# ndas7/Parallel-Systems-MPI-TFIDF

Hardware: AMD Instinct MI355X
Metric: corpus GB/s (TF-IDF hot path: tokenize->TF->DF->tf*idf->ordered output) (higher is better)
Workload: dtype u8/u32 (f64 score)

## Files before the change

parallel-systems-mpi-tfidf_amd/csrc/tokcount_sl.hip:

```cpp
#include "dev_common.h"
#include "dev_vocab.h"
#include "kernels.h"

#if defined(SL_ABL_NOVOCAB) || defined(SL_ABL_NOCOUNT) || defined(SL_ABL_NOROUNDS) || defined(SL_ABL_NOWRITE) || \
    defined(SL_ABL_NOALLOC) || defined(SL_ABL_L2C)
#define SL_ABL 1
#else
#define SL_ABL 0
#endif
#ifdef SL_ABL_NOALLOC
#define SL_ABL_ST 0
#else
#define SL_ABL_ST SL_ABL
#endif

namespace {

#ifndef SL_NT
#define SL_NT 256
#endif
constexpr int NT = SL_NT;
constexpr int NWAVE = NT / 64;
#ifndef SL_WGCU
#define SL_WGCU 4
#endif
constexpr int WG_PER_CU = SL_WGCU;
constexpr int WSTEP = 992;
#ifndef SL_TB
#define SL_TB 3584
#endif
constexpr int TB = SL_TB;
constexpr int EPT = TB / NT;
constexpr uint32_t BW = 8;
constexpr uint32_t NB = TB / BW;
constexpr uint32_t WAVE_CLAIMS = (TB - 2 * NT - 64) / NWAVE;
constexpr int GCAP = 256;
constexpr int TLW = 192;
constexpr uint32_t LEN_LONG = 31u;
constexpr uint32_t SLOT_BITS = 25;
constexpr int PMAX = 16;
#ifdef SL_STAMPS
constexpr int SL_NPH = 12;
#endif

struct SlShared {
    uint32_t TK[TB];
    uint32_t TC[TB];
    int32_t gdoc[GCAP + 1];
    uint32_t dsz[GCAP];
    union {
        struct {
            uint4 stage[NWAVE][64];
            uint32_t tl[NWAVE][TLW];
        } w;
        struct {
            uint32_t dcnt[GCAP];
            uint32_t doff[GCAP];
            uint32_t drun[GCAP];
            uint8_t dstate[GCAP];
        } f;
        struct {
            uint32_t wtot[NWAVE * 4];
            uint4 lrank[NT];
        } q;
    };
    uint4 sel[16];
    uint32_t lbase[8];
    uint32_t fl_nrec, fl_npart;
    uint8_t dpart[GCAP];
    uint8_t dfull[GCAP];
    uint32_t wsum[NWAVE];
    unsigned long long rec_base, part_base;
    unsigned long long next_chunk;
    uint32_t step_next;
};

typedef unsigned int u32x4 __attribute__((ext_vector_type(4)));
typedef unsigned int u32x4u __attribute__((ext_vector_type(4), aligned(1)));

#define RSRC_WORD3 0x00020000

template <int AUX> __device__ __forceinline__ uint4 bload16(__amdgpu_buffer_rsrc_t r, int32_t off) {
    const u32x4 v = __builtin_bit_cast(u32x4, __builtin_amdgcn_raw_buffer_load_b128(r, off, 0, AUX));
    return make_uint4(v.x, v.y, v.z, v.w);
}

__device__ __forceinline__ uint32_t zero_bits(uint32_t x) { return ~(((x & 0x7F7F7F7Fu) + 0x7F7F7F7Fu) | x) & 0x80808080u; }
__device__ __forceinline__ uint32_t compress4(uint32_t m) {
    m >>= 7;
    m |= m >> 7;
    m |= m >> 14;
    return m & 0xFu;
}

__device__ __forceinline__ uint32_t ws_flags4(uint32_t x, uint32_t& lt9) {
    const uint32_t y = x & 0x7F7F7F7Fu;
    const uint32_t a = y + 0x77777777u;
    const uint32_t b = y + 0x72727272u;
    const uint32_t c = (y ^ 0x20202020u) + 0x7F7F7F7Fu;
    lt9 |= ~(a | x) & 0x80808080u;
    return ((a & ~b) | ~c) & ~x & 0x80808080u;
}
__device__ __forceinline__ uint32_t ws_mask16_dot(uint4 v, uint32_t& lt9) {
    const uint32_t f0 = ws_flags4(v.x, lt9), f1 = ws_flags4(v.y, lt9);
    const uint32_t f2 = ws_flags4(v.z, lt9), f3 = ws_flags4(v.w, lt9);
    const uint32_t lo = __builtin_amdgcn_udot4(f0, 0x08040201u, __builtin_amdgcn_udot4(f1, 0x80402010u, 0u, false), false);
    const uint32_t hi = __builtin_amdgcn_udot4(f2, 0x08040201u, __builtin_amdgcn_udot4(f3, 0x80402010u, 0u, false), false);
    return (lo + (hi << 8)) >> 7;
}

__device__ __forceinline__ uint32_t outside16(int32_t pos, int32_t lo, int32_t hi) {
    const int32_t a = lo - pos, b = hi - pos;
    const uint32_t am = a <= 0 ? 0u : (a >= 16 ? 0xFFFFu : ((1u << a) - 1u));
    const uint32_t bm = b <= 0 ? 0u : (b >= 16 ? 0xFFFFu : ((1u << b) - 1u));
    return ~(bm & ~am) & 0xFFFFu;
}

__device__ __forceinline__ uint32_t bkt_hash(uint32_t key) {
    return __umulhi(key * 0x9E3779B1u, NB);
}
struct BktK {
    uint4 a, b;
};
__device__ __forceinline__ uint32_t bkt_slot(uint32_t b, uint32_t j) { return BW * b + j; }
__device__ __forceinline__ BktK bkt_read(const uint32_t* TK, uint32_t b) {
    const uint4* t = reinterpret_cast<const uint4*>(TK) + 2 * b;
    BktK k;
    k.a = t[0];
    k.b = t[1];
    return k;
}
__device__ __forceinline__ uint32_t bkt_match(const BktK& kk, uint32_t key) {
    uint32_t j = kk.a.x == key ? 0u : kk.a.y == key ? 1u : kk.a.z == key ? 2u : kk.a.w == key ? 3u : 8u;
    if (j == 8u) j = kk.b.x == key ? 4u : kk.b.y == key ? 5u : kk.b.z == key ? 6u : kk.b.w == key ? 7u : 8u;
    return j;
}
__device__ __forceinline__ uint32_t bkt_occ(const BktK& kk) {
    const uint32_t ta = __builtin_amdgcn_perm(kk.a.y, kk.a.x, 0x0C0C0703u) | __builtin_amdgcn_perm(kk.a.w, kk.a.z, 0x07030C0Cu);
    const uint32_t tb = __builtin_amdgcn_perm(kk.b.y, kk.b.x, 0x0C0C0703u) | __builtin_amdgcn_perm(kk.b.w, kk.b.z, 0x07030C0Cu);
    return __builtin_amdgcn_udot4(ta & 0x80808080u, 0x08040201u,
                                  __builtin_amdgcn_udot4(tb & 0x80808080u, 0x80402010u, 0u, false), false) >> 7;
}
__device__ __forceinline__ uint32_t bkt_pref(uint32_t key) { return (key * 0x85EBCA77u) >> 29; }
__device__ __forceinline__ uint32_t bkt_pick(uint32_t occ, uint32_t p) {
    const uint32_t e = ~occ & 0xFFu;
    const uint32_t r = ((e | (e << 8)) >> p) & 0xFFu;
    return r ? ((p + (uint32_t)__builtin_ctz(r)) & (BW - 1u)) : BW;
}

__device__ __noinline__ void overflow_record(const K1Out* o, uint32_t doc, uint32_t slot) {
    const uint64_t am = __ballot(1);
    const uint32_t rank = __builtin_amdgcn_mbcnt_hi((uint32_t)(am >> 32), __builtin_amdgcn_mbcnt_lo((uint32_t)am, 0u));
    unsigned long long b = 0;
    if (rank == 0u) b = gatomic_add(o->part_alloc, (unsigned long long)__popcll(am));
    const unsigned long long q = (((unsigned long long)(uint32_t)__builtin_amdgcn_readfirstlane((int)(b >> 32)) << 32) |
                                  (uint32_t)__builtin_amdgcn_readfirstlane((int)(uint32_t)b)) + rank;
    if (SL_ABL) return;
    if (q < o->part_cap) { gmem(o->part_doc)[q] = doc; gmem(o->part_slot)[q] = slot; gmem(o->part_cnt)[q] = 1u; }
    else atomicOr(o->status, ST_PART_FULL);
}

__device__ __noinline__ uint32_t bkt_slow(uint32_t* TK, uint32_t* TC, uint8_t* dpart, const K1Out* o, uint32_t key,
                                          uint32_t b, bool over, uint32_t gd0, uint32_t sb) {
    for (int probe = 0, tries = 0; probe < PMAX && tries < 64; ++tries) {
        const BktK kk = bkt_read(TK, b);
        const uint32_t j = bkt_match(kk, key);
        if (j < BW) { atomicAdd(&TC[bkt_slot(b, j)], 1u); return 0u; }
        const uint32_t e = bkt_pick(bkt_occ(kk), bkt_pref(key));
        if (e < BW) {
            if (over) break;
            const uint32_t old = atomicCAS(&TK[bkt_slot(b, e)], 0u, key);
            if (old == 0u || old == key) {
                atomicAdd(&TC[bkt_slot(b, e)], 1u);
                return old == 0u ? 1u : 0u;
            }
            continue;
        }
        b = b + 1 == NB ? 0u : b + 1;
        ++probe;
    }
    const uint32_t rel = (key & 0x7FFFFFFFu) >> sb;
    dpart[rel] = 1;
    overflow_record(o, gd0 + rel, key & ((1u << sb) - 1u));
    return 0u;
}

__device__ __noinline__ uint32_t resolve_slow(const uint8_t* __restrict__ bytes, uint4* keys, uint64_t* reps,
                                              uint64_t mask, uint32_t* status, uint32_t kind, uint32_t k0,
                                              uint32_t k1, uint32_t k2, uint32_t k3, uint64_t p0, uint64_t dend) {
    if (kind == 1u)
        return vocab_insert_s(keys, reps, mask, ((uint64_t)k1 << 32) | k0, ((uint64_t)k3 << 32) | k2, 0, status);
    uint64_t p = p0;
    while (p < dend && !is_ws(bytes[p])) ++p;
    uint64_t n = 0;
    while (p0 + n < p && bytes[p0 + n] != 0) ++n;
    uint64_t klo, khi;
    if (n < 16) {
        uint64_t lo = 0, hi = 0;
        for (uint32_t k = 0; k < n; ++k) {
            const uint64_t b = bytes[p0 + k];
            if (k < 8) lo |= b << (8 * k); else hi |= b << (8 * (k - 8));
        }
        make_short_key(lo, hi, (uint32_t)n, &klo, &khi);
        return vocab_insert_s(keys, reps, mask, klo, khi, 0, status);
    }
    make_long_key(bytes + p0, n, &klo, &khi);
    if (n > 0xFFFFFFull) atomicOr(status, ST_TERM_LONG);
    const uint64_t rep = ((n < 0xFFFFFFull ? n : 0xFFFFFFull) << 40) | p0;
    return vocab_insert_s(keys, reps, mask, klo, khi, rep, status, bytes);
}

__device__ __forceinline__ void wave_agg_add(uint32_t* ctr, uint32_t idx) {
    const uint32_t i0 = (uint32_t)__builtin_amdgcn_readfirstlane((int)idx);
    const uint64_t am = __ballot(1);
    if (__ballot(idx != i0) == 0ull) {
        if (__builtin_amdgcn_mbcnt_hi((uint32_t)(am >> 32), __builtin_amdgcn_mbcnt_lo((uint32_t)am, 0u)) == 0u)
            atomicAdd(&ctr[i0], (uint32_t)__popcll(am));
    } else {
        atomicAdd(&ctr[idx], 1u);
    }
}
__device__ __forceinline__ uint32_t wave_agg_add_rtn(uint32_t* ctr, uint32_t idx) {
    const uint32_t i0 = (uint32_t)__builtin_amdgcn_readfirstlane((int)idx);
    const uint64_t am = __ballot(1);
    uint32_t k;
    if (__ballot(idx != i0) == 0ull) {
        const uint32_t rank = __builtin_amdgcn_mbcnt_hi((uint32_t)(am >> 32), __builtin_amdgcn_mbcnt_lo((uint32_t)am, 0u));
        uint32_t b = 0;
        if (rank == 0u) b = atomicAdd(&ctr[i0], (uint32_t)__popcll(am));
        k = (uint32_t)__builtin_amdgcn_readfirstlane((int)b) + rank;
    } else {
        k = atomicAdd(&ctr[idx], 1u);
    }
    return k;
}

__device__ __forceinline__ void sl_write_staged(SlShared& S, const K1Out* o, uint32_t gd0, uint32_t sb, uint32_t nrec,
                                                uint32_t npart, unsigned long long rb, unsigned long long pb,
                                                bool rec_ok, bool part_ok) {
    const int tid = threadIdx.x;
    uint32_t* const rec_slot = o->rec_slot;
    uint32_t* const rec_cnt = o->rec_cnt;
    uint32_t* const part_doc = o->part_doc;
    uint32_t* const part_slot = o->part_slot;
    uint32_t* const part_cnt = o->part_cnt;
    const uint32_t smask = (1u << sb) - 1u;
    lds_barrier();
    if (rec_ok && !SL_ABL_ST)
        for (uint32_t i = (uint32_t)tid; i < nrec; i += NT) {
            gmem(rec_slot)[rb + i] = S.TK[i] & smask;
            gmem(rec_cnt)[rb + i] = S.TC[i];
        }
    if (part_ok && !SL_ABL_ST)
        for (uint32_t i = (uint32_t)tid; i < npart; i += NT) {
            const uint32_t k = S.TK[nrec + i];
            gmem(part_doc)[pb + i] = gd0 + ((k & 0x7FFFFFFFu) >> sb);
            gmem(part_slot)[pb + i] = k & smask;
            gmem(part_cnt)[pb + i] = S.TC[nrec + i];
        }
    lds_barrier();
    uint4* t = reinterpret_cast<uint4*>(S.TK);
#pragma unroll
    for (int j = tid; j < 2 * TB / 4; j += NT) t[j] = make_uint4(0, 0, 0, 0);
}

__device__ __forceinline__ void sl_flush(SlShared& S, const K1Out* o, uint32_t gd0, uint32_t ng, uint32_t sb) {
    const int tid = threadIdx.x;
    lds_barrier();
    if (tid < GCAP) { S.f.dcnt[tid] = 0; S.f.drun[tid] = 0; }
    lds_barrier();
    uint32_t ek[EPT], ec[EPT];
#pragma unroll
    for (int j = 0; j < EPT; ++j) {
        ek[j] = S.TK[j * NT + tid];
        ec[j] = S.TC[j * NT + tid];
        if (ek[j]) wave_agg_add(&S.f.dcnt[0], (ek[j] & 0x7FFFFFFFu) >> sb);
    }
    lds_barrier();
    uint32_t packed = 0;
    if ((uint32_t)tid < ng) {
        uint8_t st = 0;
        const uint32_t cnt = S.f.dcnt[tid];
        const bool part = S.dpart[tid] != 0;
        if (cnt) {
            const bool complete = !part && S.dfull[tid] && cnt <= (uint32_t)K5_MAX_PAIRS;
            st = complete ? 2 : 1;
            packed = complete ? cnt : (cnt << 16);
        }
        if ((st == 1 || part) && !SL_ABL) gmem(o->doc_flags)[gd0 + tid] = DF_PARTIAL;
        S.f.dstate[tid] = st;
    }
    uint32_t tot;
    const uint32_t off = block_excl_scan<NT, true>(packed, S.wsum, &tot);
    if ((uint32_t)tid < ng) S.f.doff[tid] = off;
    const uint32_t nrec = tot & 0xFFFFu, npart = tot >> 16;
    if (tid == 0) {
        const unsigned long long rb = (nrec && !SL_ABL) ? gatomic_add(o->rec_alloc, (unsigned long long)nrec) : 0ull;
        if (rb + nrec > o->rec_cap) atomicOr(o->status, ST_REC_FULL);
        S.rec_base = rb;
    } else if (tid == 64) {
        const unsigned long long pb = (npart && !SL_ABL) ? gatomic_add(o->part_alloc, (unsigned long long)npart) : 0ull;
        if (pb + npart > o->part_cap) atomicOr(o->status, ST_PART_FULL);
        S.part_base = pb;
    }
    lds_barrier();
    const unsigned long long rb = S.rec_base, pb = S.part_base;
    const bool rec_ok = rb + nrec <= o->rec_cap, part_ok = pb + npart <= o->part_cap;
    if ((uint32_t)tid < ng && S.f.dstate[tid] == 2) {
        gmem(o->doc_recoff)[gd0 + tid] = rb + (off & 0xFFFFu);
        gmem(o->doc_npairs)[gd0 + tid] = SL_ABL ? 0u : S.f.dcnt[tid];
    }
#pragma unroll
    for (int j = 0; j < EPT; ++j) {
        const uint32_t key = ek[j];
        if (key) {
            const uint32_t rel = (key & 0x7FFFFFFFu) >> sb;
            const uint32_t k = wave_agg_add_rtn(&S.f.drun[0], rel);
            const uint32_t dof = S.f.doff[rel];
            const uint32_t loc = (S.f.dstate[rel] == 2 ? (dof & 0xFFFFu) : nrec + (dof >> 16)) + k;
            S.TK[loc] = key;
            S.TC[loc] = ec[j];
        }
    }
    sl_write_staged(S, o, gd0, sb, nrec, npart, rb, pb, rec_ok, part_ok);
}

constexpr uint32_t FEW = 8;
#ifdef SL_STAMPS
#define SLF_STAMP(k)                                                        \
    do {                                                                    \
        const unsigned long long t_ = __builtin_amdgcn_s_memtime();         \
        st_acc[k] += t_ - st_t;                                             \
        st_t = t_;                                                          \
    } while (0)
#define SLF_ARGS , unsigned long long* st_acc, unsigned long long& st_t
#else
#define SLF_STAMP(k) do {} while (0)
#define SLF_ARGS
#endif
__device__ __forceinline__ void sl_flush_few(SlShared& S, const K1Out* o, uint32_t gd0, uint32_t ng, uint32_t sb SLF_ARGS) {
    const int tid = threadIdx.x;
    const int lane = tid & 63, w = tid >> 6;
    lds_barrier();
    uint32_t ek[EPT], ec[EPT];
    uint32_t c4 = 0;
#pragma unroll
    for (int j = 0; j < EPT; ++j) {
        ek[j] = S.TK[j * NT + tid];
        ec[j] = S.TC[j * NT + tid];
        c4 += (ek[j] >> 31) << (4u * ((ek[j] & 0x7FFFFFFFu) >> sb));
    }
    static_assert(EPT < 16 && FEW == 8, "4-bit per-document entry counts of eight documents");
    uint32_t pk[FEW / 2], inc[FEW / 2];
#pragma unroll
    for (uint32_t q = 0; q < FEW / 2; ++q) {
        pk[q] = ((c4 >> (8u * q)) & 15u) | (((c4 >> (8u * q + 4u)) & 15u) << 16);
        inc[q] = wave_incl_scan(pk[q]);
        if (lane == 63) S.q.wtot[w * (FEW / 2) + q] = inc[q];
    }
    SLF_STAMP(9);
    lds_barrier();
    uint32_t rank[FEW / 2], tot[FEW / 2];
#pragma unroll
    for (uint32_t q = 0; q < FEW / 2; ++q) {
        uint32_t base = 0, t = 0;
#pragma unroll
        for (int k = 0; k < NWAVE; ++k) {
            const uint32_t x = S.q.wtot[k * (FEW / 2) + q];
            base += k < w ? x : 0u;
            t += x;
        }
        rank[q] = base + inc[q] - pk[q];
        tot[q] = t;
    }
    if (w == 0) {
        const uint32_t d = (uint32_t)lane;
        uint32_t cnt = 0, packed = 0;
        uint8_t st = 0;
        if (d < ng) {
#pragma unroll
            for (uint32_t q = 0; q < FEW / 2; ++q)
                if ((d >> 1) == q) cnt = (tot[q] >> (16 * (d & 1u))) & 0xFFFFu;
            const bool part = S.dpart[d] != 0;
            if (cnt) {
                const bool complete = !part && S.dfull[d] && cnt <= (uint32_t)K5_MAX_PAIRS;
                st = complete ? 2 : 1;
                packed = complete ? cnt : (cnt << 16);
            }
            if ((st == 1 || part) && !SL_ABL) gmem(o->doc_flags)[gd0 + d] = DF_PARTIAL;
        }
        const uint32_t incl = wave_incl_scan(packed);
        const uint32_t all = (uint32_t)__builtin_amdgcn_readlane((int)incl, 63);
        const uint32_t off = incl - packed;
        const uint32_t nrec = all & 0xFFFFu, npart = all >> 16;
        unsigned long long a0 = 0, a1 = 0;
        if (lane == 0 && nrec && !SL_ABL) a0 = gatomic_add(o->rec_alloc, (unsigned long long)nrec);
        if (lane == 32 && npart && !SL_ABL) a1 = gatomic_add(o->part_alloc, (unsigned long long)npart);
        const unsigned long long rb = ((unsigned long long)(uint32_t)__builtin_amdgcn_readlane((int)(a0 >> 32), 0) << 32) |
                                      (uint32_t)__builtin_amdgcn_readlane((int)(uint32_t)a0, 0);
        const unsigned long long pb = ((unsigned long long)(uint32_t)__builtin_amdgcn_readlane((int)(a1 >> 32), 32) << 32) |
                                      (uint32_t)__builtin_amdgcn_readlane((int)(uint32_t)a1, 32);
        const bool rec_ok = rb + nrec <= o->rec_cap, part_ok = pb + npart <= o->part_cap;
        if (lane == 0 && !rec_ok) atomicOr(o->status, ST_REC_FULL);
        if (lane == 0 && !part_ok) atomicOr(o->status, ST_PART_FULL);
        if (d < ng && st == 2) {
            gmem(o->doc_recoff)[gd0 + d] = rb + (off & 0xFFFFu);
            gmem(o->doc_npairs)[gd0 + d] = SL_ABL ? 0u : cnt;
        }
        if (d < FEW) S.lbase[d] = d >= ng ? 0u : (st == 2 ? (off & 0xFFFFu) : nrec + (off >> 16));
        if (lane == 0) {
            S.fl_nrec = nrec;
            S.fl_npart = npart;
            S.rec_base = rec_ok ? rb : ~0ull;
            S.part_base = part_ok ? pb : ~0ull;
        }
    }
    lds_barrier();
    SLF_STAMP(10);
    {
        const uint4 lb0 = *reinterpret_cast<const uint4*>(&S.lbase[0]);
        const uint4 lb1 = *reinterpret_cast<const uint4*>(&S.lbase[4]);
        S.q.lrank[tid] = make_uint4(rank[0] + (lb0.x | (lb0.y << 16)), rank[1] + (lb0.z | (lb0.w << 16)),
                                    rank[2] + (lb1.x | (lb1.y << 16)), rank[3] + (lb1.z | (lb1.w << 16)));
    }
    const uint16_t* const lr16 = reinterpret_cast<const uint16_t*>(&S.q.lrank[tid]);
    uint32_t run = 0;
#pragma unroll
    for (int j = 0; j < EPT; ++j) {
        const uint32_t key = ek[j];
        if (key) {
            const uint32_t rel4 = 4u * ((key & 0x7FFFFFFFu) >> sb);
            const uint32_t loc = (uint32_t)lr16[rel4 >> 2] + ((run >> rel4) & 15u);
            run += 1u << rel4;
            S.TK[loc] = key;
            S.TC[loc] = ec[j];
        }
    }
    const unsigned long long rb = S.rec_base, pb = S.part_base;
    sl_write_staged(S, o, gd0, sb, S.fl_nrec, S.fl_npart, rb, pb, rb != ~0ull, pb != ~0ull);
}

#ifdef SL_STAMPS
#define SL_STC , st_cnt
#define SL_STC_ARG , unsigned long long* st_cnt
#else
#define SL_STC
#define SL_STC_ARG
#endif
__device__ __forceinline__ void lds_count(SlShared& S, const K1Out* o, uint32_t key, uint32_t& wclaims, uint32_t gd0,
                                          uint32_t sb SL_STC_ARG) {
    const bool over = wclaims >= WAVE_CLAIMS;
    const uint32_t b = bkt_hash(key);
    const BktK kk = bkt_read(S.TK, b);
    const bool m0 = kk.a.x == key, m1 = kk.a.y == key, m2 = kk.a.z == key, m3 = kk.a.w == key;
    const bool m4 = kk.b.x == key, m5 = kk.b.y == key, m6 = kk.b.z == key, m7 = kk.b.w == key;
    const uint32_t j = ((m1 | m3 | m5 | m7) ? 1u : 0u) | ((m2 | m3 | m6 | m7) ? 2u : 0u) | ((m4 | m5 | m6 | m7) ? 4u : 0u);
    const bool found = m0 | m1 | m2 | m3 | m4 | m5 | m6 | m7;
    const uint32_t pref = bkt_pref(key);
    uint32_t occ = bkt_occ(kk);
    const uint32_t n = bkt_pick(occ, pref);
    const bool hit = key != 0u && found;
    const bool claim = key != 0u && !found && n < BW && !over;
    const uint32_t idx = bkt_slot(b, found ? j : (n & (BW - 1u)));
    const uint32_t old = atomicCAS(&S.TK[idx], hit ? key : (claim ? 0u : 0x7FFFFFFFu), key);
    const bool ok = key != 0u && (old == key || (claim && old == 0u));
    atomicAdd(&S.TC[idx], ok ? 1u : 0u);
    bool claimed = claim && old == 0u;
    bool slow = key != 0u && !ok;
#ifdef SL_STAMPS
    st_cnt[0] += __ballot(slow) != 0ull ? 1u : 0u;
    st_cnt[1] += (uint32_t)__popcll(__ballot(slow));
    st_cnt[2] += (uint32_t)__popcll(__ballot(claim && !ok));
    ++st_cnt[4];
#endif
    uint32_t nn = n;
#pragma unroll
    for (int t = 0; t < 2; ++t) {
        if (claim && slow) {
            occ |= 1u << (nn & (BW - 1u));
            nn = bkt_pick(occ, pref);
        }
        const bool lost = claim && slow && nn < BW;
        if (__ballot(lost) == 0ull) break;
        if (lost) {
            const uint32_t i2 = bkt_slot(b, nn);
            const uint32_t o2 = atomicCAS(&S.TK[i2], 0u, key);
            if (o2 == 0u || o2 == key) {
                atomicAdd(&S.TC[i2], 1u);
                slow = false;
                claimed = o2 == 0u;
            }
        }
    }
    {
        const bool full = slow && !claim && !over && key != 0u;
        if (__ballot(full) != 0ull) {
            if (full) {
                const uint32_t b2 = b + 1u == NB ? 0u : b + 1u;
                const BktK k2 = bkt_read(S.TK, b2);
                const uint32_t j2 = bkt_match(k2, key);
                uint32_t e2 = j2;
                bool ok2 = j2 < BW;
                if (!ok2) {
                    e2 = bkt_pick(bkt_occ(k2), pref);
                    if (e2 < BW) {
                        const uint32_t o2 = atomicCAS(&S.TK[bkt_slot(b2, e2)], 0u, key);
                        ok2 = o2 == 0u || o2 == key;
                        claimed = o2 == 0u;
                    }
                }
                if (ok2) {
                    atomicAdd(&S.TC[bkt_slot(b2, e2)], 1u);
                    slow = false;
                }
            }
        }
    }
#ifdef SL_STAMPS
    st_cnt[3] += __ballot(slow) != 0ull ? 1u : 0u;
    st_cnt[5] += (uint32_t)__popcll(__ballot(slow && claim));
    st_cnt[6] += (uint32_t)__popcll(__ballot(slow && !claim && !over));
    st_cnt[7] += (uint32_t)__popcll(__ballot(slow && over));
#endif
    uint32_t claims = claimed ? 1u : 0u;
    if (__ballot(slow) != 0ull) {
        if (slow) claims = bkt_slow(S.TK, S.TC, S.dpart, o, key, b, over, gd0, sb);
    }
    wclaims += (uint32_t)__popcll(__ballot(claims != 0u));
}

__device__ __forceinline__ uint32_t perm_sel(uint32_t n, uint32_t k) {
    uint32_t s = 0;
    for (uint32_t j = 0; j < 4; ++j) {
        const uint32_t p = 4 * k + j;
        const uint32_t b = p < n ? j : (p == n ? 4u : 12u);
        s |= b << (8 * j);
    }
    return s;
}

struct Round {
    uint32_t k0, k1, k2, k3;
    uint32_t h;
    uint32_t rel, kind;
    int32_t ap;
#ifdef SL_DEBUG
    uint32_t ent;
#endif
    uint4 s0, s1;
};

}

__global__ __launch_bounds__(NT, WG_PER_CU * NT / 256) void k_tokcount_sl(CorpusDev c, const uint64_t* __restrict__ chunk_start,
                                                               const uint32_t* __restrict__ chunk_doc, uint64_t c0,
                                                               uint64_t c1, VocabDev v, const K1Out* __restrict__ o,
                                                               uint32_t sb, uint32_t gcap) {
    __shared__ __attribute__((aligned(16))) SlShared S;
    const int tid = threadIdx.x, lane = tid & 63;
    const int wid = __builtin_amdgcn_readfirstlane(tid >> 6);
    unsigned long long tokens_w = 0;
    bool clean = false;
#ifdef SL_STAMPS
    unsigned long long st_acc[SL_NPH] = {};
    unsigned long long st_t = __builtin_amdgcn_s_memtime(), st_chunks = 0;
    unsigned long long st_cnt[8] = {};
#define SL_STAMP(k)                                                         \
    do {                                                                    \
        const unsigned long long t_ = __builtin_amdgcn_s_memtime();         \
        st_acc[k] += t_ - st_t;                                             \
        st_t = t_;                                                          \
    } while (0)
#else
#define SL_STAMP(k) do {} while (0)
#endif
    if (tid == 0) S.next_chunk = c0 + gatomic_add(o->chunk_ctr, 1ull);
    lds_barrier();
    unsigned long long claim = 0;
    for (uint64_t chunk = (uint64_t)__builtin_amdgcn_readfirstlane((int)(uint32_t)S.next_chunk) |
                          ((uint64_t)__builtin_amdgcn_readfirstlane((int)(uint32_t)(S.next_chunk >> 32)) << 32);
         chunk < c1;) {
    if (tid == 0) claim = c0 + gatomic_add(o->chunk_ctr, 1ull);
    const uint64_t cs = chunk_start[chunk], ce = chunk_start[chunk + 1];
    const uint32_t dfirst = chunk_doc[chunk], dlast = chunk_doc[chunk + 1];
#ifdef SL_STAMPS
    ++st_chunks;
#endif
    if (cs < ce) {

    const uint64_t b0 = cs & ~(uint64_t)15;
    const uint64_t rb = b0 >= 16 ? b0 - 16 : 0;
    const int32_t shift = (int32_t)(b0 - rb);
    const uint64_t avail = c.nbytes > rb ? ((c.nbytes - rb + 15) & ~(uint64_t)15) : 0;
    const __amdgpu_buffer_rsrc_t crs = __builtin_amdgcn_make_buffer_rsrc(
        (void*)(c.bytes + rb), 0, (int)(avail < 0x7FFFFFF0ull ? avail : 0x7FFFFFF0ull), RSRC_WORD3);
    const __amdgpu_buffer_rsrc_t vrs = __builtin_amdgcn_make_buffer_rsrc((void*)v.keys, 0, (int)((v.mask + 1) * 16),
                                                                         RSRC_WORD3);
    const int32_t span = (int32_t)(ce - b0);
    const int32_t cs_rel = (int32_t)(cs - b0);
    const int32_t lo_rel = c.lo > b0 ? (c.lo - b0 > (uint64_t)span ? span : (int32_t)(c.lo - b0)) : -64;
    const int32_t hi_rel = c.hi - b0 > (uint64_t)span + 64 ? span + 64 : (int32_t)(c.hi - b0);

    const uint32_t ng0 = (dlast + 1 - dfirst) < gcap ? (dlast + 1 - dfirst) : gcap;
    const uint64_t dpre = (uint32_t)tid <= ng0 ? c.doc_off[dfirst + tid] : 0ull;
    uint4 pf = bload16<2>(crs, wid * WSTEP + 16 * lane - 16 + shift);
    if (!clean) {
        uint4* t = reinterpret_cast<uint4*>(S.TK);
        for (int j = tid; j < 2 * TB / 4; j += NT) t[j] = make_uint4(0, 0, 0, 0);
        if (tid < 64) {
            const uint32_t n = (uint32_t)tid >> 2, k = (uint32_t)tid & 3u;
            (&S.sel[n].x)[k] = perm_sel(n, k);
        }
        clean = true;
    }
    uint8_t* const stage = reinterpret_cast<uint8_t*>(&S.w.stage[wid][0]);
    uint32_t* const tl = S.w.tl[wid];

    for (uint32_t gd0 = dfirst; gd0 <= dlast; gd0 += gcap) {
        const uint32_t ng = (dlast + 1 - gd0) < gcap ? (dlast + 1 - gd0) : gcap;
        for (uint32_t k = tid; k <= ng; k += NT) {
            const uint64_t d = (gd0 == dfirst && k == (uint32_t)tid) ? dpre : c.doc_off[gd0 + k];
            S.gdoc[k] = d < b0 ? -64 : (d - b0 > (uint64_t)span + 64 ? span + 64 : (int32_t)(d - b0));
        }
        if (tid < GCAP) { S.dsz[tid] = 0; S.dpart[tid] = 0; }
        if (tid == 0) S.step_next = NWAVE;
        lds_barrier();
        if ((uint32_t)tid < ng) S.dfull[tid] = S.gdoc[tid] >= cs_rel && S.gdoc[tid + 1] <= span;
        const int32_t g0 = __builtin_amdgcn_readfirstlane(S.gdoc[0]);
        const int32_t gn = __builtin_amdgcn_readfirstlane(S.gdoc[ng]);
        const int32_t gs = g0 > cs_rel ? g0 : cs_rel;
        const int32_t ge = gn < span ? gn : span;
        SL_STAMP(0);

        Round pend, acc;
        pend.kind = 0;
        pend.k0 = pend.k1 = pend.k2 = pend.k3 = 0;
        pend.h = 0;
        pend.rel = 0;
        pend.ap = 0;
        pend.s0 = pend.s1 = make_uint4(0, 0, 0, 0);
#ifdef SL_DEBUG
        pend.ent = 0;
#endif
        acc = pend;
        uint32_t fill = 0;
        uint32_t wclaims = 0;

        auto promote = [&](Round& p, const Round& a) {
            p.k0 = a.k0; p.k1 = a.k1; p.k2 = a.k2; p.k3 = a.k3;
            p.h = a.h; p.rel = a.rel; p.kind = a.kind; p.ap = a.ap;
#ifdef SL_DEBUG
            p.ent = a.ent;
#endif
#ifdef SL_ABL_NOVOCAB
            p.s0 = make_uint4(p.k0, p.k1, p.k2, p.k3);
            p.s1 = p.s0;
#else
            p.s0 = bload16<0>(vrs, (int32_t)(p.h << 4));
            p.s1 = bload16<0>(vrs, (int32_t)(p.h << 4) + 16);
#endif
        };
        auto finish = [&](const Round& r) {
#ifdef SL_STAMPS
            asm volatile("s_waitcnt vmcnt(0)" ::: "memory");
            SL_STAMP(11);
#endif
            const bool h0 = ((r.s0.x ^ r.k0) | (r.s0.y ^ r.k1) | (r.s0.z ^ r.k2) | (r.s0.w ^ r.k3)) == 0u;
            const bool h1 = ((r.s1.x ^ r.k0) | (r.s1.y ^ r.k1) | (r.s1.z ^ r.k2) | (r.s1.w ^ r.k3)) == 0u;
            uint32_t slot = r.h + (h0 ? 0u : 1u);
#ifdef SL_ABL_NOVOCAB
            const bool need = false;
#else
            const bool need = (r.kind == 2u) | ((r.kind == 1u) & !(h0 | h1));
#endif
            if (__ballot(need) != 0ull) {
                if (need) {
                    const uint64_t p0 = b0 + (uint64_t)(int64_t)r.ap;
                    const uint64_t dend = c.doc_off[gd0 + r.rel + 1];
                    slot = resolve_slow(c.bytes, v.keys, v.rep, v.mask, o->status, r.kind, r.k0, r.k1, r.k2, r.k3, p0,
                                        dend);
                }
            }
            const uint32_t key = (r.kind != 0u && slot != INVALID_SLOT) ? (0x80000000u | (r.rel << sb) | slot) : 0u;
#ifdef SL_DEBUG
            if (o->stamps && r.kind != 0u) {
                const unsigned long long q = atomicAdd(&o->stamps[0], 1ull);
                if (q < (K1_DEBUG_WORDS - 8) / 4) {
                    unsigned long long* d = o->stamps + 8 + 4 * q;
                    d[0] = ((unsigned long long)r.ent << 32) | ((uint32_t)r.ap << 8) | r.kind;
                    d[1] = ((unsigned long long)r.k1 << 32) | r.k0;
                    d[2] = ((unsigned long long)r.k3 << 32) | r.k2;
                    d[3] = ((unsigned long long)key << 32) | slot;
                }
            }
#endif
#ifdef SL_ABL_NOCOUNT
            wclaims += (uint32_t)__popcll(__ballot(key == 0x12345u));
            return;
#endif
            lds_count(S, o, key, wclaims, gd0, sb SL_STC);
        };
        auto build = [&](Round& a, uint32_t e, int32_t sbp) {
            const uint32_t pos = e & 1023u, len = (e >> 10) & 31u;
            a.rel = e >> 16;
            a.ap = sbp - 16 + (int32_t)pos;
            a.kind = len >= 16u ? 2u : 1u;
#ifdef SL_DEBUG
            a.ent = e;
#endif
            const u32x4u raw = *reinterpret_cast<const u32x4u*>(stage + pos);
            const uint4 sl = S.sel[len & 15u];
            a.k0 = __builtin_amdgcn_perm(0x09090909u, raw.x, sl.x);
            a.k1 = __builtin_amdgcn_perm(0x09090909u, raw.y, sl.y);
            a.k2 = __builtin_amdgcn_perm(0x09090909u, raw.z, sl.z);
            a.k3 = __builtin_amdgcn_perm(0x09090909u, raw.w, sl.w);
            a.h = (uint32_t)key_hash(((uint64_t)a.k1 << 32) | a.k0, ((uint64_t)a.k3 << 32) | a.k2) & (uint32_t)v.mask & ~1u;
        };
        auto turn = [&]() {
            finish(pend);
            promote(pend, acc);
            acc.kind = 0u;
            fill = 0u;
        };

        if (gs < ge) {
            const int32_t bs = gs & ~15;
            const int32_t nsteps = (ge - bs + WSTEP - 1) / WSTEP;
            const bool inner_all = bs >= lo_rel + 16 && bs + nsteps * WSTEP + 16 <= hi_rel;
            if (gd0 != dfirst || bs != 0) pf = bload16<2>(crs, bs + wid * WSTEP + 16 * lane - 16 + shift);
            uint32_t wr = 0;
            int32_t wcur = g0, wnext = ng > 1 ? __builtin_amdgcn_readfirstlane(S.gdoc[1]) : gn;
            for (int32_t s = wid, snext = wid; s < nsteps; s = snext) {
                {
                    uint32_t nx = 0;
                    if (lane == 0) nx = atomicAdd(&S.step_next, 1u);
                    snext = __builtin_amdgcn_readfirstlane((int)nx);
                }
                const int32_t sbp = bs + s * WSTEP;
                const int32_t gpos = sbp + 16 * lane - 16;
                const uint4 cur = pf;
#ifdef SL_ABL_L2C
                pf = bload16<2>(crs, bs + (snext & 3) * WSTEP + 16 * lane - 16 + shift);
#else
                pf = bload16<2>(crs, bs + snext * WSTEP + 16 * lane - 16 + shift);
#endif
                reinterpret_cast<uint4*>(stage)[lane] = cur;
                uint32_t lt9 = 0;
                uint32_t ws = ws_mask16_dot(cur, lt9);
                if (!inner_all) ws |= outside16(gpos, lo_rel, hi_rel);
                while (wr + 1 < ng && wnext <= sbp) {
                    ++wr;
                    wcur = wnext;
                    wnext = __builtin_amdgcn_readfirstlane(S.gdoc[wr + 1]);
                }
                uint32_t ds = 0, base = wr;
                const bool multi = wnext < sbp + WSTEP + 16 || wcur + 16 >= sbp;
                if (multi) {
                    for (uint32_t k = wr; k <= ng; ++k) {
                        const int32_t sk = __builtin_amdgcn_readfirstlane(S.gdoc[k]);
                        if (sk >= sbp + WSTEP + 16) break;
                        base += (k > wr && sk < gpos) ? 1u : 0u;
                        if (sk >= gpos && sk < gpos + 16) ds |= 1u << (uint32_t)(sk - gpos);
                    }
                }
                const uint32_t prev = (lane_prev(ws) >> 15) & 1u;
                uint32_t own = (lane >= 1 && lane <= 62) ? 0xFFFFu : 0u;
                if (!(sbp >= gs && sbp + WSTEP <= ge) && own) own &= ~outside16(gpos, gs, ge);
                const uint32_t starts = ~ws & ((ws << 1) | prev | ds) & own & 0xFFFFu;
                uint32_t nul = 0;
                const bool nulany = __ballot(lt9 != 0u) != 0ull;
                if (nulany)
                    nul = compress4(zero_bits(cur.x)) | (compress4(zero_bits(cur.y)) << 4) |
                          (compress4(zero_bits(cur.z)) << 8) | (compress4(zero_bits(cur.w)) << 12);
                const uint32_t stop = ws | ds;
                const uint32_t stop32 = stop | (lane_next(stop) << 16), nul32 = nul | (lane_next(nul) << 16);
                const uint32_t nmine = (uint32_t)__popc(starts);
                const uint32_t incl = wave_incl_scan(nmine);
                const uint32_t ntok = (uint32_t)__builtin_amdgcn_readlane((int)incl, 63);
                SL_STAMP(1);
                if (ntok == 0) continue;
                tokens_w += ntok;
#ifdef SL_ABL_NOROUNDS
                if (!multi && lane == 0) atomicAdd(&S.dsz[wr], ntok);
                continue;
#endif
                if (!multi && lane == 0) atomicAdd(&S.dsz[wr], ntok);
                const bool fast = !multi && !nulany && ntok <= (uint32_t)TLW;
                for (uint32_t tb = 0; tb < ntok; tb += TLW) {
                    if (fast) {
                        const uint32_t eb = ((uint32_t)lane << 4) | (wr << 16), s32 = stop32 | 0x80000000u;
                        uint32_t sm = starts;
                        uint32_t* p = tl + (incl - nmine);
                        while (sm) {
                            const uint32_t i = __builtin_ctz(sm);
                            sm &= sm - 1;
                            *p++ = eb | i | ((uint32_t)__builtin_ctz(s32 >> i) << 10);
                        }
                    } else {
                        uint32_t sm = starts, idx = incl - nmine;
                        while (sm) {
                            const uint32_t i = __builtin_ctz(sm);
                            sm &= sm - 1;
                            if (idx - tb < (uint32_t)TLW) {
                                const uint32_t e = ((stop32 >> i) & ~1u) | (nul32 >> i);
                                const uint32_t len = e ? (uint32_t)__builtin_ctz(e) : LEN_LONG;
                                uint32_t rel = base;
                                if (ds & ((2u << i) - 1u))
                                    while (rel + 1 < ng && S.gdoc[rel + 1] <= gpos + (int32_t)i) ++rel;
                                tl[idx - tb] = ((uint32_t)lane << 4 | i) | ((len < 16u ? len : LEN_LONG) << 10) | (rel << 16);
                                if (multi) atomicAdd(&S.dsz[rel], 1u);
                            }
                            ++idx;
                        }
                    }
                    __builtin_amdgcn_fence(__ATOMIC_RELEASE, "wavefront");
                    __builtin_amdgcn_wave_barrier();
                    __builtin_amdgcn_fence(__ATOMIC_ACQUIRE, "wavefront");
                    const uint32_t cnt = (ntok - tb) < (uint32_t)TLW ? (ntok - tb) : (uint32_t)TLW;
                    SL_STAMP(2);
                    for (uint32_t t = 0; t < cnt;) {
                        const uint32_t m = (64u - fill) < (cnt - t) ? (64u - fill) : (cnt - t);
                        if ((uint32_t)lane >= fill && (uint32_t)lane < fill + m) {
                            const uint32_t e = tl[t + (uint32_t)lane - fill];
                            build(acc, e, sbp);
                        }
                        t += m;
                        fill += m;
                        if (fill == 64u) {
                            SL_STAMP(3);
                            turn();
                            SL_STAMP(4);
                        }
                    }
                    __builtin_amdgcn_fence(__ATOMIC_RELEASE, "wavefront");
                    __builtin_amdgcn_wave_barrier();
                    __builtin_amdgcn_fence(__ATOMIC_ACQUIRE, "wavefront");
                }
            }
        }
        SL_STAMP(3);
        if (fill) turn();
        finish(pend);
#ifdef SL_STAMPS
        SL_STAMP(5);
        lds_barrier();
        SL_STAMP(7);
#endif
#ifdef SL_STAMPS
        if (ng <= FEW) sl_flush_few(S, o, gd0, ng, sb, st_acc, st_t);
#else
        if (ng <= FEW) sl_flush_few(S, o, gd0, ng, sb);
#endif
        else sl_flush(S, o, gd0, ng, sb);
        if ((uint32_t)tid < ng) {
            const uint32_t n = S.dsz[tid];
            if (n) {
                if (S.dfull[tid]) gmem(o->doc_size)[gd0 + tid] = n;
                else atomicAdd(&o->doc_size[gd0 + tid], n);
            }
        }
        lds_barrier();
        SL_STAMP(8);
        if (gd0 + gcap < gd0) break;
    }
    }
    if (tid == 0) S.next_chunk = claim;
    lds_barrier();
    chunk = (uint64_t)(uint32_t)__builtin_amdgcn_readfirstlane((int)(uint32_t)S.next_chunk) |
            ((uint64_t)(uint32_t)__builtin_amdgcn_readfirstlane((int)(uint32_t)(S.next_chunk >> 32)) << 32);
    SL_STAMP(6);
    }
    if (lane == 0 && tokens_w) atomicAdd(o->ntokens, tokens_w);
#ifdef SL_STAMPS
    SL_STAMP(6);
    if (lane == 0 && o->stamps) {
        for (int k = 0; k < SL_NPH; ++k) atomicAdd(&o->stamps[k], st_acc[k]);
        atomicAdd(&o->stamps[SL_NPH], st_chunks);
        atomicAdd(&o->stamps[SL_NPH + 1], 1ull);
        for (int k = 0; k < 8; ++k) atomicAdd(&o->stamps[SL_NPH + 2 + k], st_cnt[k]);
    }
#endif
}

int launch_tokcount_sl(const CorpusDev& c, const uint64_t* chunk_start, const uint32_t* chunk_doc, uint64_t c0,
                       uint64_t c1, const VocabDev& v, const K1Out* o_dev, hipStream_t s) {
    if (c1 <= c0) return 0;
    if (v.mask >= (1ull << SLOT_BITS)) return -3;
    static_assert(sizeof(SlShared) * WG_PER_CU <= 163840, "LDS of WG_PER_CU workgroups per CU");
    static_assert(TB % NT == 0 && TB % BW == 0, "table rows");
    const uint32_t sbits = (uint32_t)__builtin_popcountll(v.mask);
    const uint32_t gcap = (1u << (31u - sbits)) >= (uint32_t)GCAP ? (uint32_t)GCAP : (1u << (31u - sbits));
    static int ncu = 0;
    if (!ncu) {
        int dev = 0;
        if (hipGetDevice(&dev) != hipSuccess ||
            hipDeviceGetAttribute(&ncu, hipDeviceAttributeMultiprocessorCount, dev) != hipSuccess || ncu <= 0)
            ncu = 256;
    }
    const uint64_t wgs = (uint64_t)ncu * WG_PER_CU;
    const uint64_t grid = (c1 - c0) < wgs ? (c1 - c0) : wgs;
    k_tokcount_sl<<<(unsigned)grid, NT, 0, s>>>(c, chunk_start, chunk_doc, c0, c1, v, o_dev, sbits, gcap);
    return hipGetLastError() == hipSuccess ? 0 : -1;
}
```

Measured before the change: 331.3.

## Add single-probe fast path with per-wave pending queue for LDS token counting

Adds a FAST variant of the LDS hash-count step. Each key first tries a single CAS at its preferred bucket slot, and keys that miss are pushed into a per-wave LDS queue. Once 64 keys are queued they go through the full 8-way bucket probe together, and leftovers are drained at the end of each chunk. Claim accounting changes from a per-wave budget to a workgroup-wide sum published in LDS. This aims to cut the bucket-read and divergent slow-path cost on common keys, at the price of extra LDS, fences and possible table-fill imbalance.

```diff
diff --git a/parallel-systems-mpi-tfidf_amd/csrc/tokcount_sl.hip b/parallel-systems-mpi-tfidf_amd/csrc/tokcount_sl.hip
--- a/parallel-systems-mpi-tfidf_amd/csrc/tokcount_sl.hip
+++ b/parallel-systems-mpi-tfidf_amd/csrc/tokcount_sl.hip
@@ -39,6 +39,7 @@
 constexpr uint32_t LEN_LONG = 31u;
 constexpr uint32_t SLOT_BITS = 25;
 constexpr int PMAX = 16;
+constexpr uint32_t PQ = 128;
 #ifdef SL_STAMPS
 constexpr int SL_NPH = 12;
 #endif
@@ -73,6 +74,8 @@
     unsigned long long rec_base, part_base;
     unsigned long long next_chunk;
     uint32_t step_next;
+    uint32_t pq[NWAVE][PQ];
+    uint32_t wcl[NWAVE];
 };
 
 typedef unsigned int u32x4 __attribute__((ext_vector_type(4)));
@@ -447,9 +450,24 @@
 #define SL_STC
 #define SL_STC_ARG
 #endif
-__device__ __forceinline__ void lds_count(SlShared& S, const K1Out* o, uint32_t key, uint32_t& wclaims, uint32_t gd0,
-                                          uint32_t sb SL_STC_ARG) {
-    const bool over = wclaims >= WAVE_CLAIMS;
+template <bool FAST> __device__ __forceinline__ bool claims_over(SlShared& S, uint32_t wclaims) {
+    if (wclaims < WAVE_CLAIMS) return false;
+    if (!FAST) return true;
+    const uint32_t w = threadIdx.x >> 6;
+    uint32_t sum = wclaims;
+#pragma unroll
+    for (uint32_t k = 0; k < (uint32_t)NWAVE; ++k)
+        sum += k == w ? 0u : __hip_atomic_load(&S.wcl[k], __ATOMIC_RELAXED, __HIP_MEMORY_SCOPE_WORKGROUP);
+    return sum >= (uint32_t)NWAVE * WAVE_CLAIMS;
+}
+__device__ __forceinline__ void claims_publish(SlShared& S, uint32_t wclaims) {
+    __hip_atomic_store(&S.wcl[threadIdx.x >> 6], wclaims, __ATOMIC_RELAXED, __HIP_MEMORY_SCOPE_WORKGROUP);
+}
+
+template <bool FAST>
+__device__ __forceinline__ uint32_t lds_count_full(SlShared& S, const K1Out* o, uint32_t key, uint32_t wclaims, uint32_t gd0,
+                                                uint32_t sb SL_STC_ARG) {
+    const bool over = claims_over<FAST>(S, wclaims);
     const uint32_t b = bkt_hash(key);
     const BktK kk = bkt_read(S.TK, b);
     const bool m0 = kk.a.x == key, m1 = kk.a.y == key, m2 = kk.a.z == key, m3 = kk.a.w == key;
@@ -526,7 +544,60 @@
     if (__ballot(slow) != 0ull) {
         if (slow) claims = bkt_slow(S.TK, S.TC, S.dpart, o, key, b, over, gd0, sb);
     }
-    wclaims += (uint32_t)__popcll(__ballot(claims != 0u));
+    return wclaims + (uint32_t)__popcll(__ballot(claims != 0u));
+}
+
+__device__ __forceinline__ void pq_fence() {
+    __builtin_amdgcn_fence(__ATOMIC_RELEASE, "wavefront");
+    __builtin_amdgcn_wave_barrier();
+    __builtin_amdgcn_fence(__ATOMIC_ACQUIRE, "wavefront");
+}
+
+template <bool FAST>
+__device__ __forceinline__ void lds_count(SlShared& S, const K1Out* o, uint32_t key, uint32_t& wclaims, uint32_t& npend,
+                                          uint32_t* pq, uint32_t gd0, uint32_t sb SL_STC_ARG) {
+    if (!FAST) {
+        wclaims = lds_count_full<false>(S, o, key, wclaims, gd0, sb SL_STC);
+        return;
+    }
+    static_assert(NWAVE * 64 <= NT + 64, "claim overshoot inside WAVE_CLAIMS' margin");
+    const bool over = claims_over<FAST>(S, wclaims);
+    const uint32_t idx = bkt_slot(bkt_hash(key), bkt_pref(key));
+    const uint32_t old = atomicCAS(&S.TK[idx], (key != 0u && !over) ? 0u : 0x7FFFFFFFu, key);
+    const bool ok = key != 0u && (old == key || (!over && old == 0u));
+    atomicAdd(&S.TC[idx], ok ? 1u : 0u);
+    const uint64_t cm = __ballot(ok && old == 0u);
+    const bool slow = key != 0u && !ok;
+    wclaims += (uint32_t)__popcll(cm);
+    const uint64_t sm = __ballot(slow);
+#ifdef SL_STAMPS
+    ++st_cnt[8];
+    st_cnt[9] += (uint32_t)__popcll(__ballot(ok && old != 0u));
+    st_cnt[10] += (uint32_t)__popcll(cm);
+    st_cnt[11] += (uint32_t)__popcll(sm);
+#endif
+    if (sm != 0ull) {
+        if (slow) pq[npend + __builtin_amdgcn_mbcnt_hi((uint32_t)(sm >> 32), __builtin_amdgcn_mbcnt_lo((uint32_t)sm, 0u))] = key;
+        npend += (uint32_t)__popcll(sm);
+        if (npend >= 64u) {
+            pq_fence();
+            npend -= 64u;
+            claims_publish(S, wclaims);
+            wclaims = lds_count_full<true>(S, o, pq[npend + (threadIdx.x & 63u)], wclaims, gd0, sb SL_STC);
+        }
+    }
+    claims_publish(S, wclaims);
+}
+template <bool FAST>
+__device__ __forceinline__ void lds_drain(SlShared& S, const K1Out* o, uint32_t& wclaims, uint32_t& npend, uint32_t* pq,
+                                          uint32_t gd0, uint32_t sb SL_STC_ARG) {
+    while (npend) {
+        pq_fence();
+        const uint32_t m = npend < 64u ? npend : 64u, l = threadIdx.x & 63u;
+        npend -= m;
+        wclaims = lds_count_full<FAST>(S, o, l < m ? pq[npend + l] : 0u, wclaims, gd0, sb SL_STC);
+        claims_publish(S, wclaims);
+    }
 }
 
 __device__ __forceinline__ uint32_t perm_sel(uint32_t n, uint32_t k) {
@@ -552,6 +623,7 @@
 
 }
 
+template <bool FAST>
 __global__ __launch_bounds__(NT, WG_PER_CU * NT / 256) void k_tokcount_sl(CorpusDev c, const uint64_t* __restrict__ chunk_start,
                                                                const uint32_t* __restrict__ chunk_doc, uint64_t c0,
                                                                uint64_t c1, VocabDev v, const K1Out* __restrict__ o,
@@ -564,7 +636,7 @@
 #ifdef SL_STAMPS
     unsigned long long st_acc[SL_NPH] = {};
     unsigned long long st_t = __builtin_amdgcn_s_memtime(), st_chunks = 0;
-    unsigned long long st_cnt[8] = {};
+    unsigned long long st_cnt[12] = {};
 #define SL_STAMP(k)                                                         \
     do {                                                                    \
         const unsigned long long t_ = __builtin_amdgcn_s_memtime();         \
@@ -624,6 +696,7 @@
         }
         if (tid < GCAP) { S.dsz[tid] = 0; S.dpart[tid] = 0; }
         if (tid == 0) S.step_next = NWAVE;
+        if (tid < NWAVE) S.wcl[tid] = 0;
         lds_barrier();
         if ((uint32_t)tid < ng) S.dfull[tid] = S.gdoc[tid] >= cs_rel && S.gdoc[tid + 1] <= span;
         const int32_t g0 = __builtin_amdgcn_readfirstlane(S.gdoc[0]);
@@ -645,6 +718,8 @@
         acc = pend;
         uint32_t fill = 0;
         uint32_t wclaims = 0;
+        uint32_t npend = 0;
+        uint32_t* const pq = S.pq[wid];
 
         auto promote = [&](Round& p, const Round& a) {
             p.k0 = a.k0; p.k1 = a.k1; p.k2 = a.k2; p.k3 = a.k3;
@@ -698,7 +773,7 @@
             wclaims += (uint32_t)__popcll(__ballot(key == 0x12345u));
             return;
 #endif
-            lds_count(S, o, key, wclaims, gd0, sb SL_STC);
+            lds_count<FAST>(S, o, key, wclaims, npend, pq, gd0, sb SL_STC);
         };
         auto build = [&](Round& a, uint32_t e, int32_t sbp) {
             const uint32_t pos = e & 1023u, len = (e >> 10) & 31u;
@@ -841,6 +916,7 @@
         SL_STAMP(3);
         if (fill) turn();
         finish(pend);
+        lds_drain<FAST>(S, o, wclaims, npend, pq, gd0, sb SL_STC);
 #ifdef SL_STAMPS
         SL_STAMP(5);
         lds_barrier();
@@ -877,7 +953,7 @@
         for (int k = 0; k < SL_NPH; ++k) atomicAdd(&o->stamps[k], st_acc[k]);
         atomicAdd(&o->stamps[SL_NPH], st_chunks);
         atomicAdd(&o->stamps[SL_NPH + 1], 1ull);
-        for (int k = 0; k < 8; ++k) atomicAdd(&o->stamps[SL_NPH + 2 + k], st_cnt[k]);
+        for (int k = 0; k < 12; ++k) atomicAdd(&o->stamps[SL_NPH + 2 + k], st_cnt[k]);
     }
 #endif
 }
@@ -899,6 +975,9 @@
     }
     const uint64_t wgs = (uint64_t)ncu * WG_PER_CU;
     const uint64_t grid = (c1 - c0) < wgs ? (c1 - c0) : wgs;
-    k_tokcount_sl<<<(unsigned)grid, NT, 0, s>>>(c, chunk_start, chunk_doc, c0, c1, v, o_dev, sbits, gcap);
+    if (v.mask + 1 > K1_ST_MAX_CAP)
+        k_tokcount_sl<false><<<(unsigned)grid, NT, 0, s>>>(c, chunk_start, chunk_doc, c0, c1, v, o_dev, sbits, gcap);
+    else
+        k_tokcount_sl<true><<<(unsigned)grid, NT, 0, s>>>(c, chunk_start, chunk_doc, c0, c1, v, o_dev, sbits, gcap);
     return hipGetLastError() == hipSuccess ? 0 : -1;
 }
```

After: 339.9, median of 6. +2.6%, better.
